# duyhominhnguyen/conan-fgw

Measured on AMD Instinct MI355X. Metric: molecules/s (K=5 conformers), higher is better.
Workload: dtype f32

## Files before the change

### conan-fgw_amd/csrc/fgw_small.hip

```cpp
#include "fgw_common.h"

#ifdef CONAN_FGW_PROFILE
FGW_PROF_ACCESSOR(conan_debug_fgw_prof)
FGW_PROF_TRACE_ACCESSOR(conan_debug_fgw_trace)
#endif

namespace {

constexpr int SK_SCRATCH_DOUBLES = 3 * 256 + 2 * 64;

template <int R, bool KL, bool SECOND = false>
__global__ void __launch_bounds__(FGW_THREADS, (SECOND || R > 9) ? 1 : 3) k_fgw_coupling_small(
    const float *__restrict__ Ys, const float *__restrict__ Cs, const float *__restrict__ ps, const float *__restrict__ pb,
    FgwDims D, conan_fgw_params prm, int outer, int y_zero, const double *__restrict__ Cw, const double *__restrict__ Yw,
    const int *__restrict__ active, float *__restrict__ Tw, int *__restrict__ info, fgw_part_t *__restrict__ Ypart,
    fgw_part_t *__restrict__ Cpart, const double *__restrict__ zvec, const double *__restrict__ yvec, const int *__restrict__ only, FgwAdj adj) {
    extern __shared__ __attribute__((aligned(16))) char smem[];
    auto solve = [&](const int cid) {
    const int b = cid / D.K, s = cid % D.K;
    if (!fgw_active(active, D.B, b, outer)) return;
    const int N = D.N, P = D.P, d = D.d;
    const int NN = N * N, NP = N * P;
    const int tid = threadIdx.x, lane = tid & 63, w = __builtin_amdgcn_readfirstlane(tid >> 6);
    const bool lane_ok = lane < N;
    FGW_PROF_DECL;

    double *Al = reinterpret_cast<double *>(smem);
    double *Gl = Al + NP;
    double *C1l = Gl + NP;
    double *Bl = C1l + NP;
    double *pq = Bl + NP;
    double *red = pq + 128;
    float *t_dummy = reinterpret_cast<float *>(red + 7);
    double *vec4 = red + 8;
    const bool alias = (size_t)NP >= SK_SCRATCH_DOUBLES;
    double *own = vec4 + 256;
    double *bufC = alias ? Al : own;
    double *bufK = bufC + 256;
    double *bufR = bufK + 256;
    double *fcp = bufR + 256;
    double *gcp = fcp + 64;
    float *Tl = reinterpret_cast<float *>(own + (alias ? 0 : SK_SCRATCH_DOUBLES));
    float *C2l = Tl + NP;
    double *Yl = Al;
    float *Zl = reinterpret_cast<float *>(Bl);
    float *Zl2 = reinterpret_cast<float *>(Gl);
    const bool yz_lds = d <= 2 * P;
    const bool z_lds = (size_t)N * d * sizeof(float) <= (size_t)NP * sizeof(double);

    const float *Z = Ys + ((size_t)b * D.K + s) * N * d;
    const float *C2 = adj.rowptr ? adj_dense_slice<FGW_THREADS>(adj, cid, N, tid) : Cs + ((size_t)b * D.K + s) * NN;
    const double *C1 = Cw + (size_t)b * NN;
    const double *Y = Yw + (size_t)b * N * d;
    float *Tg = Tw + ((size_t)b * D.K + s) * NN;
    const double alpha = (double)prm.alpha, inv_eps = 1.0 / (double)prm.epsilon;

    constexpr int EPT = (16 * R * R + FGW_THREADS - 1) / FGW_THREADS;
    double c1v[EPT];
    float c2v[EPT], tv[EPT];
    const bool warm = outer > 0 && prm.warmstart;
#pragma unroll
    for (int u = 0; u < EPT; ++u) {
        const int t = tid + u * FGW_THREADS, tc = t < NN ? t : NN - 1;
        c1v[u] = C1[tc]; c2v[u] = C2[tc]; tv[u] = warm ? Tg[tc] : 0.f;
    }
    const double p_own = tid < N ? (pb ? (double)pb[(size_t)b * N + tid] : 1.0 / (double)N) : 1.0;
    const double q_own = tid < N ? (ps ? (double)ps[((size_t)b * D.K + s) * N + tid] : 1.0 / (double)N) : 1.0;
    double vec_own;
    {
        const int v = tid >> 6, i = tid & 63;
        const double *src = (v == 0 || v == 2) ? yvec + (size_t)b * 2 * N + (v == 0 ? N : 0) : zvec + ((size_t)b * D.K + s) * 2 * N + (v == 1 ? N : 0);
        vec_own = src[i < N ? i : N - 1];
        vec_own = i < N ? vec_own : 0.0;
    }
    const bool stage_yz = yz_lds && !y_zero;
    if (stage_yz) {
        const int Nd = N * d;
        for (int t0 = tid; t0 < Nd; t0 += 4 * FGW_THREADS) {
            double yv[4]; float zv[4];
#pragma unroll
            for (int u = 0; u < 4; ++u) { const int t = t0 + u * FGW_THREADS, tc = t < Nd ? t : Nd - 1; yv[u] = Y[tc]; zv[u] = Z[tc]; }
#pragma unroll
            for (int u = 0; u < 4; ++u) { const int t = t0 + u * FGW_THREADS; if (t < Nd) { Yl[t] = yv[u]; Zl[t] = zv[u]; } }
        }
    }
    if (tid < 64) { pq[tid] = p_own; pq[64 + tid] = q_own; }
    const bool massless = __syncthreads_or(tid < N && (p_own <= 0.0 || q_own <= 0.0)) != 0;
    vec4[tid] = vec_own;
#pragma unroll
    for (int u = 0; u < EPT; ++u) {
        const int t = tid + u * FGW_THREADS;
        if (t < NN) { const int i = t / N, j = t - i * N; C2l[i * P + j] = c2v[u]; if (!stage_yz) C1l[i * P + j] = c1v[u]; }
    }
    __syncthreads();
    FGW_PROF(0);
    const double qj = pq[64 + lane];
    const double pi_l = pq[lane];
#pragma unroll
    for (int u = 0; u < EPT; ++u) {
        const int t = tid + u * FGW_THREADS;
        if (t < NN) { const int i = t / N, j = t - i * N; Tl[i * P + j] = warm ? tv[u] : (float)(pq[i] * pq[64 + j]); }
    }
    const double *r1v = vec4, *r2v = vec4 + 64, *y2v = vec4 + 128, *z2v = vec4 + 192;
    double *Dl = stage_yz ? C1l : Al;
    if (!y_zero) {
        if (stage_yz)
            mm_lds<FGW_WAVES, true>(N, N, d, Yl, d, Zl, d, [&](int i, int j, double v) { Dl[i * P + j] = v; }, border_prepare(N, N));
        else
            mm_f64(N, N, d, [&](int i, int k) { return Y[(size_t)i * d + k]; }, [&](int k, int j) { return (double)Z[(size_t)j * d + k]; },
                   [&](int i, int j, double v) { Dl[i * P + j] = v; });
    }
    __syncthreads();
    FGW_PROF(1);
#pragma unroll
    for (int u = 0; u < EPT; ++u) {
        const int t = tid + u * FGW_THREADS;
        if (t < NN) {
            const int i = t / N, j = t - i * N;
            double m = -2.0 * (y_zero ? 0.0 : Dl[i * P + j]); m += y2v[i]; m += z2v[j];
            m = m > 0.0 ? m : 0.0;
            Bl[i * P + j] = 2.0 * alpha * (r1v[i] + r2v[j]) + (1.0 - alpha) * m;
        }
    }
    __syncthreads();
    if (stage_yz) {
#pragma unroll
        for (int u = 0; u < EPT; ++u) {
            const int t = tid + u * FGW_THREADS;
            if (t < NN) { const int i = t / N, j = t - i * N; C1l[i * P + j] = c1v[u]; }
        }
        __syncthreads();
    }
    FGW_PROF(2);

    const BorderIdx bnn = border_prepare(N, N);
    int cpt = 0, sk_total = 0;
    double err = 1.0;
    while (err > (double)prm.inner_tol && cpt < prm.max_iter) {
        mm_lds<FGW_WAVES, false>(N, N, N, C1l, P, Tl, P, [&](int i, int j, double v) { Al[i * P + j] = v; }, bnn);
        __syncthreads();
        FGW_PROF(3);
        auto product_G = [&]() {
            if constexpr (KL)
                mm_f64(N, N, N, [&](int i, int k) { return Al[i * P + k]; }, [&](int k, int j) { return log((double)C2l[j * P + k] + 1e-15); },
                       [&](int i, int j, double v) { Gl[i * P + j] = v; }, bnn);
            else
                mm_lds<FGW_WAVES, true>(N, N, N, Al, P, C2l, P, [&](int i, int j, double v) { Gl[i * P + j] = 2.0 * v; }, bnn);
        };
        product_G();
        __syncthreads();
        FGW_PROF(4);
        int lq = lane, wq = w;
        asm volatile("" : "+v"(lq), "+v"(wq));
        const int lc = lq < N ? lq : N - 1;
        auto mrA = [&](int r) { const int q = wq + 4 * r, qc = q < N ? q : N - 1; const double m = -(Bl[qc * P + lc] - 2.0 * alpha * Gl[qc * P + lc]) * inv_eps; return (q < N && lane_ok) ? m : -1.0e300; };
        auto mrB = [&](int r) { const int q = wq + 4 * r, qc = q < N ? q : N - 1; const double m = -(Bl[lc * P + qc] - 2.0 * alpha * Gl[lc * P + qc]) * inv_eps; return (q < N && lane_ok) ? m : -1.0e300; };
        double kA[R], kB[R];
        int ii = 0;
        bool exact = massless;
        {
            const double ref_own = -(Bl[lc * P + lc] - 2.0 * alpha * Gl[lc * P + lc]) * inv_eps;
            fcp[lane] = ref_own;
            double cs = 0.0;
#pragma unroll
            for (int r = 0; r < R; ++r) { kA[r] = exp_fast(mrA(r) - ref_own); cs += kA[r]; }
            bufK[w * 64 + lane] = cs;
#pragma unroll
            for (int r = 0; r < R; ++r) { const int q = wq + 4 * r; kB[r] = exp_fast(mrB(r) - fcp[q < N ? q : N - 1]); }
            __syncthreads();
            cs = ((bufK[lane] + bufK[64 + lane]) + bufK[128 + lane]) + bufK[192 + lane];
            if (__any(lane_ok && !(cs > 1e-150 && cs < 1e150))) exact = true;
            const double f = lane_ok ? qj * rcp_pos(cs) : 0.0;
            gcp[lane] = f;
#pragma unroll
            for (int r = 0; r < R; ++r) { kA[r] *= f; kB[r] *= gcp[w + 4 * r]; }
        }
        FGW_PROF(5);
        double colsum = 0.0;
        bool have_colsum = false;
        for (; !exact && ii < prm.num_iter_max; ++ii) {
            if (ii > 0) {
                if (!have_colsum) {
                    double cs = 0.0;
#pragma unroll
                    for (int r = 0; r < R; ++r) cs += kA[r];
                    bufC[w * 64 + lane] = cs;
                    __syncthreads();
                    colsum = ((bufC[lane] + bufC[64 + lane]) + bufC[128 + lane]) + bufC[192 + lane];
                }
                have_colsum = false;
                if (__any(lane_ok && !(colsum > 1e-150 && colsum < 1e150))) { exact = true; break; }
                const double f = lane_ok ? qj * rcp_pos(colsum) : 0.0;
                fcp[lane] = f;
#pragma unroll
                for (int r = 0; r < R; ++r) { kA[r] *= f; kB[r] *= fcp[w + 4 * r]; }
            }
            double rs = 0.0;
#pragma unroll
            for (int r = 0; r < R; ++r) rs += kB[r];
            bufR[w * 64 + lane] = rs;
            __syncthreads();
            rs = ((bufR[lane] + bufR[64 + lane]) + bufR[128 + lane]) + bufR[192 + lane];
            if (__any(lane_ok && !(rs > 1e-150 && rs < 1e150))) { exact = true; break; }
            const double g = lane_ok ? pi_l * rcp_pos(rs) : 0.0;
            gcp[lane] = g;
#pragma unroll
            for (int r = 0; r < R; ++r) { kB[r] *= g; kA[r] *= gcp[w + 4 * r]; }
            if (ii % 10 == 0) {
                double cs = 0.0;
#pragma unroll
                for (int r = 0; r < R; ++r) cs += kA[r];
                bufK[w * 64 + lane] = cs;
                __syncthreads();
                colsum = ((bufK[lane] + bufK[64 + lane]) + bufK[128 + lane]) + bufK[192 + lane];
                have_colsum = true;
                double df = lane_ok ? colsum - qj : 0.0;
                df = wave_sum_d(df * df);
                if (sqrt(df) < (double)prm.stop_thr) { ++ii; break; }
            }
        }
        if (exact) {
            __syncthreads();
            double *xm = bufC, *xs = bufK, *uc = fcp, *vc = gcp;
            const double loga = log(pi_l), logb = log(qj);
            double u_l = 0.0, v_l = 0.0;
            uc[lane] = (lane_ok && !(pi_l > 0.0)) ? loga : 0.0;
            for (ii = 0; ii < prm.num_iter_max; ++ii) {
                double z[R];
                double mx = -1.0e300;
#pragma unroll
                for (int r = 0; r < R; ++r) { z[r] = mrA(r) + uc[w + 4 * r]; mx = fmax(z[r], mx); }
                double sm = 0.0;
#pragma unroll
                for (int r = 0; r < R; ++r) sm += exp_lse(z[r] - mx);
                __syncthreads();
                xm[w * 64 + lane] = mx; xs[w * 64 + lane] = sm;
                __syncthreads();
                {
                    const double m0 = xm[lane], m1 = xm[64 + lane], m2 = xm[128 + lane], m3 = xm[192 + lane];
                    const double M = fmax(fmax(m0, m1), fmax(m2, m3));
                    sm = ((xs[lane] * exp_lse(m0 - M) + xs[64 + lane] * exp_lse(m1 - M)) + xs[128 + lane] * exp_lse(m2 - M)) +
                         xs[192 + lane] * exp_lse(m3 - M);
                    v_l = lane_ok ? logb - (log_acc(sm) + M) : 0.0;
                }
                vc[lane] = v_l;
                mx = -1.0e300;
#pragma unroll
                for (int r = 0; r < R; ++r) { z[r] = mrB(r) + vc[w + 4 * r]; mx = fmax(z[r], mx); }
                sm = 0.0;
#pragma unroll
                for (int r = 0; r < R; ++r) sm += exp_lse(z[r] - mx);
                __syncthreads();
                xm[w * 64 + lane] = mx; xs[w * 64 + lane] = sm;
                __syncthreads();
                {
                    const double m0 = xm[lane], m1 = xm[64 + lane], m2 = xm[128 + lane], m3 = xm[192 + lane];
                    const double M = fmax(fmax(m0, m1), fmax(m2, m3));
                    sm = ((xs[lane] * exp_lse(m0 - M) + xs[64 + lane] * exp_lse(m1 - M)) + xs[128 + lane] * exp_lse(m2 - M)) +
                         xs[192 + lane] * exp_lse(m3 - M);
                    u_l = lane_ok ? loga - (log_acc(sm) + M) : 0.0;
                }
                uc[lane] = u_l;
                if (ii % 10 == 0) {
                    double cs = 0.0;
#pragma unroll
                    for (int r = 0; r < R; ++r) cs += exp_acc(mrA(r) + uc[w + 4 * r] + v_l);
                    __syncthreads();
                    xs[w * 64 + lane] = cs;
                    __syncthreads();
                    cs = ((xs[lane] + xs[64 + lane]) + xs[128 + lane]) + xs[192 + lane];
                    double df = lane_ok ? cs - qj : 0.0;
                    df = wave_sum_d(df * df);
                    if (sqrt(df) < (double)prm.stop_thr) { ++ii; break; }
                }
            }
#pragma unroll
            for (int r = 0; r < R; ++r) kA[r] = exp_acc(mrA(r) + uc[w + 4 * r] + v_l);
        }
        sk_total += ii;
        FGW_PROF(6);
        double e2 = 0.0;
#pragma unroll
        for (int r = 0; r < R; ++r) {
            const int i = wq + 4 * r;
            const bool ok = lane_ok && i < N;
            float *tp = ok ? &Tl[i * P + lq] : t_dummy;
            const float tn = (float)kA[r];
            const double df = ok ? (double)tn - (double)*tp : 0.0;
            e2 += df * df;
            *tp = tn;
        }
        if (cpt % 10 == 0) err = sqrt(block_sum_d(e2, red));
        else __syncthreads();
        ++cpt;
        FGW_PROF(7);
    }
    __syncthreads();
    for (int t = tid; t < NN; t += FGW_THREADS) { const int i = t / N, j = t - i * N; Tg[t] = Tl[i * P + j]; }
    if (tid == 0) { atomicAdd(&info[b * 4 + 1], cpt); atomicAdd(&info[b * 4 + 2], sk_total); }
    FGW_PROF(8);

    if (!prm.fixed_features && Ypart) {
// ... 233 lines not shown
        __syncthreads();
        nb = max(max(ired[0], ired[1]), max(ired[2], ired[3]));
        __syncthreads();
        pad_ok = pad_try && N - nb >= 2 && nb >= 1;
        if (pad_ok) pad_ok = c1_block_ok(nb);
    }
    int m_pad = 0;
    if (pad_try && N - nb >= 2 && nb >= 1) {
        auto nearf = [](double a, double b_) { return fabs(a - b_) <= 1e-9 * (fabs(b_) + 1e-30) || a == b_; };
        bool ok = pad_ok;
        for (int r = nb + 1 + w; r < N; r += FGW_WAVES)
            for (int c = lane; c < d; c += 64) {
                if (stage_yz) {
                    ok = ok && nearf((double)Zl[r * d + c], (double)Zl[nb * d + c]) && nearf(Yl[r * d + c], Yl[nb * d + c]);
                } else {
                    ok = ok && nearf((double)Z[(size_t)r * d + c], (double)Z[(size_t)nb * d + c]);
                    if (!y_zero) ok = ok && nearf(Y[(size_t)r * d + c], Y[(size_t)nb * d + c]);
                }
            }
        if (__syncthreads_and(ok) != 0) m_pad = N - nb;
    }
    const int Nx = m_pad ? nb + 1 : N;
    const double mult = m_pad ? (double)m_pad : 1.0;
    FGW_PROF(0);
    const double qj = pq[64 + lane] * ((m_pad && lane == nb) ? mult : 1.0);
    const double pi_l = pq[lane] * ((m_pad && lane == nb) ? mult : 1.0);
    const double *r1v = vec4, *r2v = vec4 + 64, *y2v = vec4 + 128, *z2v = vec4 + 192;
    auto base_of = [&](int i, int j, double dot) {
        double m = -2.0 * dot; m += y2v[i]; m += z2v[j];
        m = m > 0.0 ? m : 0.0;
        return fc.two_alpha * (r1v[i] + r2v[j]) + fc.one_m_alpha * m;
    };
    if (y_zero) {
        int i = e_i0, j = e_j0;
#pragma unroll
        for (int u = 0; u < EPT; ++u) {
            if (tid + u * FGW_THREADS < NN) Bl[i * P + j] = base_of(i, j, 0.0);
            j += e_dr; i += e_dq;
            if (j >= N) { j -= N; ++i; }
        }
    } else if (stage_yz) {
        mm_lds2<FGW_WAVES, MAXT, 0, true, true>(Nx, Nx, d, Yl, d, Zl, d, [&]() { load_c1_t(); __syncthreads(); },
                                                [&](int i, int j, double v) { Bl[i * P + j] = base_of(i, j, v); });
        for_entries([&](int u, int o) { C1l[o] = c1v[u]; });
    } else {
        mm_f64(Nx, Nx, d, [&](int i, int k) { return Y[(size_t)i * d + k]; }, [&](int k, int j) { return (double)Z[(size_t)j * d + k]; },
               [&](int i, int j, double v) { Bl[i * P + j] = base_of(i, j, v); });
    }
    __syncthreads();
    FGW_PROF(1);
    if (warm) {
        if (m_pad) {
            int i = e_i0, j = e_j0;
#pragma unroll
            for (int u = 0; u < EPT; ++u) {
                if (tid + u * FGW_THREADS < NN) Tl[i * P + j] = (float)((double)tv[u] * ((i == nb ? mult : 1.0) * (j == nb ? mult : 1.0)));
                j += e_dr; i += e_dq;
                if (j >= N) { j -= N; ++i; }
            }
        } else {
            for_entries([&](int u, int o) { Tl[o] = tv[u]; });
        }
    } else {
#pragma unroll
        for (int r = 0; r < R; ++r) {
            const int i = w + 4 * r;
            const double pi_r = (pb ? (double)pb[(size_t)b * N + (i < N ? i : N - 1)] : fc.inv_n) * ((m_pad && i == nb) ? mult : 1.0);
            if (i < Nx && lane < Nx) Tl[i * P + lane] = (float)(pi_r * qj);
        }
    }
    __syncthreads();
    FGW_PROF(2);

    int cpt = 0, sk_total = 0;
    double err = 1.0;
    bool bail = __syncthreads_or(tid < N && (p_own <= 0.0 || q_own <= 0.0)) != 0;
    while (!bail && err > fc.inner_tol && cpt < prm.max_iter) {
        int tq = tid, N = Nx, P = D.P;
        asm volatile("" : "+v"(tq), "+s"(N), "+s"(P));
        int nbq = m_pad ? nb : -1;
        asm volatile("" : "+s"(nbq));
        const int lq = tq & 63, wq = tq >> 6;
        const bool lq_ok = lq < N;
        mm_lds2<FGW_WAVES, 1, 0, false, false>(N, N, N, C1l, P, Tl, P, [] {}, [&](int i, int j, double v) { AKl[i * P + j] = v; }, tq);
        __syncthreads();
        FGW_PROF(3);
        int nr = n_real;
        asm volatile("" : "+s"(nr));
        if (complete) {
            {
                const int lc = lq_ok ? lq : N - 1;
                const double *ar = AKl + lc * P + wq;
                double p0 = 0.0, p1 = 0.0;
#pragma unroll
                for (int r = 0; r < R; ++r) {
                    const int q = wq + 4 * r;
                    if (q < nr) { if (r & 1) p1 += ar[4 * r]; else p0 += ar[4 * r]; }
                }
                if (lq_ok) rsum[wq * N + lq] = p0 + p1;
            }
            __syncthreads();
            {
                int i = tq / N, j = tq - i * N;
                const int dq = FGW_THREADS / N, dr = FGW_THREADS - dq * N;
                for (int t = tq; t < N * N; t += FGW_THREADS) {
                    const int o = i * P + j;
                    const double ai = ((rsum[i] + rsum[N + i]) + rsum[2 * N + i]) + rsum[3 * N + i];
                    const double v = j < nr ? ai - AKl[o] : 0.0;
                    const double x = fma(v, fc.four_alpha_inv_eps, (Bl[j * P + j] - Bl[o]) * fc.inv_eps);
                    AKl[o] = exp_fast(x);
                    j += dr; i += dq;
                    if (j >= N) { j -= N; ++i; }
                }
            }
        } else {
            mm_lds2<FGW_WAVES, MAXT, 0, true, true>(N, N, N, AKl, P, C2l, P, [&]() { __syncthreads(); }, [&](int i, int j, double v) {
                const double x = fma(v, fc.four_alpha_inv_eps, (Bl[j * P + j] - Bl[i * P + j]) * fc.inv_eps);
                AKl[i * P + j] = exp_fast(x);
            }, tq);
        }
        __syncthreads();
        FGW_PROF(4);
        double kA[R], kB[R];
        {
            const int lc = lq_ok ? lq : N - 1;
#pragma unroll
            for (int r = 0; r < R; ++r) {
                const int q = wq + 4 * r, qc = q < N ? q : N - 1;
                const double a = AKl[qc * P + lc], bb = AKl[lc * P + qc];
                const bool ok = q < N && lq_ok;
                kA[r] = ok ? a : 0.0; kB[r] = ok ? bb : 0.0;
            }
        }
        __syncthreads();
        FGW_PROF(5);
        const int permL = (lq & 3) * 16 + (lq >> 2);
        double *bufCw = bufC + wq * 64 + lq, *bufRw = bufR + wq * 64 + lq;
        const double *fw = fvP + wq * 16, *gw = gvP + wq * 16;
        auto dotR = [&](const double (&k)[R], const double *v) {
            double p0 = 0.0, p1 = 0.0, p2 = 0.0;
#pragma unroll
            for (int r = 0; r < R; ++r) {
                if (r % 3 == 0) p0 = fma(k[r], v[r], p0);
                else if (r % 3 == 1) p1 = fma(k[r], v[r], p1);
                else p2 = fma(k[r], v[r], p2);
            }
            return (p0 + p1) + p2;
        };
        int ii = 0;
        double f = 0.0, g = 0.0, colp = 0.0;
        bool have_colp = false;
        for (; ii < prm.num_iter_max; ++ii) {
            if (!have_colp) {
                double pc = 0.0;
                if (ii == 0) {
                    gvP[permL] = lq_ok ? (lq == nbq ? (double)m_pad : 1.0) : 0.0;
                }
                pc = dotR(kA, gw);
                *bufCw = pc;
                __syncthreads();
                colp = ((bufC[lq] + bufC[64 + lq]) + bufC[128 + lq]) + bufC[192 + lq];
            }
            have_colp = false;
            if (__any(lq_ok && !(colp > 1e-150 && colp < 1e150))) { bail = true; break; }
            f = lq_ok ? qj * rcp_pos(colp) : 0.0;
            fvP[permL] = f;
            *bufRw = dotR(kB, fw);
            __syncthreads();
            const double rs = ((bufR[lq] + bufR[64 + lq]) + bufR[128 + lq]) + bufR[192 + lq];
            if (__any(lq_ok && !(rs > 1e-150 && rs < 1e150))) { bail = true; break; }
            g = lq_ok ? pi_l * rcp_pos(rs) : 0.0;
            gvP[permL] = g;
            if (ii % 10 == 0) {
                *bufCw = dotR(kA, gw);
                __syncthreads();
                colp = ((bufC[lq] + bufC[64 + lq]) + bufC[128 + lq]) + bufC[192 + lq];
                have_colp = true;
                double df = lq_ok ? f * colp - qj : 0.0;
                df = df * df;
                if (lq == nbq) df /= (double)m_pad;
                df = wave_sum_d(df);
                if (sqrt(df) < fc.stop_thr) { ++ii; break; }
            }
        }
        if (bail) break;
        sk_total += ii;
        FGW_PROF(6);
        double e2 = 0.0;
        {
            float *trow = Tl + wq * P + lq;
#pragma unroll
            for (int r = 0; r < R; ++r) {
                const bool ok = lq_ok && wq + 4 * r < N;
                float *tp = ok ? trow + 4 * r * P : t_dummy;
                const float tn = (float)((gw[r] * kA[r]) * f);
                double df = ok ? (double)tn - (double)*tp : 0.0;
                df *= df;
                if (nbq >= 0) {
                    const double im = 1.0 / (double)m_pad;
                    df *= (lq == nbq ? im : 1.0) * (wq + 4 * r == nbq ? im : 1.0);
                }
                e2 += df;
                *tp = tn;
            }
        }
        if (cpt % 10 == 0) err = sqrt(block_sum_d(e2, red));
        else __syncthreads();
        ++cpt;
        FGW_PROF(7);
    }
    if (bail) {
        if (tid == 0) { redo[cid] = 1; atomicOr(&info[b * 4 + 3], 1); }
        return;
    }
    __syncthreads();
    {
        int te = tid;
        asm volatile("" : "+v"(te));
        int i = te / N, j = te - i * N;
        const int dq = FGW_THREADS / N, dr = FGW_THREADS - dq * N;
        if (m_pad) {
            const float im = (float)(1.0 / mult);
            for (int t = te; t < NN; t += FGW_THREADS) {
                Tg[t] = Tl[min(i, nb) * P + min(j, nb)] * ((i >= nb ? im : 1.0f) * (j >= nb ? im : 1.0f));
                j += dr; i += dq;
                if (j >= N) { j -= N; ++i; }
            }
        } else {
            for (int t = te; t < NN; t += FGW_THREADS) {
                Tg[t] = Tl[i * P + j];
                j += dr; i += dq;
                if (j >= N) { j -= N; ++i; }
            }
        }
    }
    if (tid == 0) { atomicAdd(&info[b * 4 + 1], cpt); atomicAdd(&info[b * 4 + 2], sk_total); redo[cid] = 0; if (m_pad) atomicOr(&info[b * 4 + 3], 2); }
    FGW_PROF(8);

    if (!prm.fixed_features && Ypart) {
        fgw_part_t *Yp = Ypart + ((size_t)b * D.K + s) * N * d;
        if (yz_lds) {
            const int Nd = N * d;
            for (int t0 = tid; t0 < Nd; t0 += 4 * FGW_THREADS) {
                float zv[4];
#pragma unroll
                for (int u = 0; u < 4; ++u) { const int t = t0 + u * FGW_THREADS; zv[u] = Z[t < Nd ? t : Nd - 1]; }
#pragma unroll
                for (int u = 0; u < 4; ++u) { const int t = t0 + u * FGW_THREADS; if (t < Nd) Zl[t] = zv[u]; }
            }
            __syncthreads();
            mm_lds2<FGW_WAVES, 1, 0, false, false>(N, d, N, Tl, P, Zl, d, [] {}, [&](int i, int c, double v) { Yp[(size_t)i * d + c] = (fgw_part_t)v; });
        } else {
            mm_f64(N, d, N, [&](int i, int k) { return (double)Tl[i * P + k]; }, [&](int k, int c) { return (double)Z[(size_t)k * d + c]; },
                   [&](int i, int c, double v) { Yp[(size_t)i * d + c] = (fgw_part_t)v; });
        }
    }
    FGW_PROF(9);
    if (!prm.fixed_structure) {
        fgw_part_t *Cp = Cpart + ((size_t)b * D.K + s) * NN;
        if (complete) {
            {
                const int lc = lane < Nx ? lane : Nx - 1;
                const float *tr = Tl + lc * P + w;
                double p0 = 0.0, p1 = 0.0;
#pragma unroll
                for (int r = 0; r < R; ++r) {
                    const int q = w + 4 * r;
                    if (q < n_real) { if (r & 1) p1 += (double)tr[4 * r]; else p0 += (double)tr[4 * r]; }
                }
                if (lane < Nx) rsum[w * N + lane] = p0 + p1;
            }
            __syncthreads();
            mm_lds2<FGW_WAVES, 1, 0, true, false>(Nx, Nx, n_real, Tl, P, Tl, P, [] {}, [&](int i, int j, double v) {
                const double ti = ((rsum[i] + rsum[N + i]) + rsum[2 * N + i]) + rsum[3 * N + i];
                const double tj = ((rsum[j] + rsum[N + j]) + rsum[2 * N + j]) + rsum[3 * N + j];
                if (m_pad) Bl[i * P + j] = ti * tj - v;
                else Cp[i * N + j] = (fgw_part_t)(ti * tj - v);
            });
        } else {
            mm_lds2<FGW_WAVES, 1, 0, false, false>(Nx, Nx, Nx, Tl, P, C2l, P, [] {}, [&](int i, int j, double v) { AKl[i * P + j] = v; });
            __syncthreads();
            mm_lds2<FGW_WAVES, 1, 0, true, false>(Nx, Nx, Nx, AKl, P, Tl, P, [] {}, [&](int i, int j, double v) {
                if (m_pad) Bl[i * P + j] = v;
                else Cp[i * N + j] = (fgw_part_t)v;
            });
        }
        if (m_pad) {
            __syncthreads();
            const double im = 1.0 / mult;
            int i = tid / N, j = tid - i * N;
            const int dq = FGW_THREADS / N, dr = FGW_THREADS - dq * N;
            for (int t = tid; t < NN; t += FGW_THREADS) {
                Cp[t] = (fgw_part_t)(Bl[min(i, nb) * P + min(j, nb)] * ((i >= nb ? im : 1.0) * (j >= nb ? im : 1.0)));
                j += dr; i += dq;
                if (j >= N) { j -= N; ++i; }
            }
        }
    }
    FGW_PROF(10);
    FGW_PROF_FLUSH;
    FGW_PROF_TRACE(Nx | (cpt << 8) | (sk_total << 20));
}

template <int NT>
__device__ __forceinline__ void molecule_vectors(const double *__restrict__ Y, const double *__restrict__ C, const float *__restrict__ p, int N,
                                                 int d, bool kl, double *__restrict__ out, int which = 2) {
    constexpr int LPI = NT / 64;
    const int i = (int)threadIdx.x / LPI, sub = (int)threadIdx.x % LPI;
    double y2 = 0.0, r1 = 0.0;
    if (i < N) {
        if (which != 1)
            for (int c = sub; c < d; c += LPI) { const double v = Y[(size_t)i * d + c]; y2 += v * v; }
        if (which != 0)
            for (int k = sub; k < N; k += LPI) {
                const double c1 = C[i * N + k], pk = p ? (double)p[k] : 1.0 / (double)N;
                r1 += (kl ? c1 * log(c1 + 1e-15) - c1 : c1 * c1) * pk;
            }
    }
#pragma unroll
    for (int o = 1; o < LPI; o <<= 1) { y2 += __shfl_xor(y2, o, 64); r1 += __shfl_xor(r1, o, 64); }
    if (i < N && sub == 0) { if (which != 1) out[i] = y2; if (which != 0) out[N + i] = r1; }
}

__global__ void __launch_bounds__(256) k_fgw_small_vectors(const float *__restrict__ Ys, const float *__restrict__ Cs, const float *__restrict__ ps,
                                                           const float *__restrict__ pb, FgwDims D, int kl, double *__restrict__ Cw,
                                                           double *__restrict__ Yw, double *__restrict__ zvec, double *__restrict__ yvec,
                                                           const float *__restrict__ init_C, const float *__restrict__ init_Y, int max_iter,
                                                           int *__restrict__ active, int *__restrict__ info, float *__restrict__ errs,
                                                           float *__restrict__ Yout, float *__restrict__ Cout, FgwAdj adj) {
    const int b = blockIdx.x / D.K, s = blockIdx.x % D.K;
    const int N = D.N, d = D.d;
    __shared__ __attribute__((aligned(16))) unsigned char cm[64 * 65 + 16];
    const int Pm = D.P;
    if (adj.rowptr) {
        for (int t = threadIdx.x; t < (64 * 65 + 16) / 4; t += 256) reinterpret_cast<unsigned *>(cm)[t] = 0u;
        __syncthreads();
        adj_scatter_lds_bytes<256>(adj, (int)blockIdx.x, N, Pm, cm, (int)threadIdx.x);
        __syncthreads();
    }
    if (s == 0) {
        const int NN = N * N, Nd = N * d;
        const float *c0 = init_C ? init_C + (size_t)b * NN : Cs + (size_t)b * D.K * NN;
        for (int t = threadIdx.x; t < NN; t += 256) {
            const float cv = (!init_C && adj.rowptr) ? (float)cm[(t / N) * Pm + (t % N)] : c0[t];
            Cw[(size_t)b * NN + t] = (double)cv; Cout[(size_t)b * NN + t] = cv;
        }
        for (int t = threadIdx.x; t < Nd; t += 256) {
            const float y = init_Y ? init_Y[(size_t)b * Nd + t] : 0.f;
            Yw[(size_t)b * Nd + t] = (double)y; Yout[(size_t)b * Nd + t] = y;
        }
        if (threadIdx.x == 0) { fgw_active_init(active, D.B, b); info[b * 4 + 0] = 0; info[b * 4 + 1] = 0; info[b * 4 + 2] = 0; info[b * 4 + 3] = 0; }
        for (int t = threadIdx.x; t < 2 * max_iter; t += 256) errs[(size_t)b * 2 * max_iter + t] = __builtin_nanf("");
        __syncthreads();
    }
    const float *Z = Ys + ((size_t)b * D.K + s) * N * d;
    const float *C2 = Cs + ((size_t)b * D.K + s) * N * N;
    const float *q = ps ? ps + ((size_t)b * D.K + s) * N : nullptr;
    const int j = (int)threadIdx.x >> 2, sub = (int)threadIdx.x & 3;
    double z2 = 0.0, r2 = 0.0;
    if (j < N) {
        for (int c = sub; c < d; c += 4) { const double v = (double)Z[(size_t)j * d + c]; z2 += v * v; }
        for (int k = sub; k < N; k += 4) {
            const double c2 = adj.rowptr ? (double)cm[j * Pm + k] : (double)C2[j * N + k], qk = q ? (double)q[k] : 1.0 / (double)N;
            r2 += qk * (kl ? c2 : c2 * c2);
        }
    }
    z2 += __shfl_xor(z2, 1, 64); z2 += __shfl_xor(z2, 2, 64);
    r2 += __shfl_xor(r2, 1, 64); r2 += __shfl_xor(r2, 2, 64);
    double *zo = zvec + ((size_t)b * D.K + s) * 2 * N;
    if (j < N && sub == 0) { zo[j] = z2; zo[N + j] = r2; }
    if (s == 0)
        molecule_vectors<256>(Yw + (size_t)b * N * d, Cw + (size_t)b * N * N, pb ? pb + (size_t)b * N : nullptr, N, d, kl != 0, yvec + (size_t)b * 2 * N);
    if (adj.order && blockIdx.x == gridDim.x - 1) fgw_order_by_size<256>(adj, D.B, D.K, (int)threadIdx.x);
}

constexpr int UPD_THREADS = 512;
template <bool Y_FROM_T>
__global__ void __launch_bounds__(UPD_THREADS) k_fgw_update_parts(
    const float *__restrict__ pb, const float *__restrict__ lambdas, FgwDims D, conan_fgw_params prm, int outer,
    const fgw_part_t *__restrict__ Ypart, const fgw_part_t *__restrict__ Cpart, double *__restrict__ Cw, double *__restrict__ Yw,
    int *__restrict__ active, int *__restrict__ info, float *__restrict__ errs, float *__restrict__ Yout, float *__restrict__ Cout,
    double *__restrict__ yvec, const float *__restrict__ Tw, const float *__restrict__ Ys, int chunk) {
    __shared__ double red[UPD_THREADS / 64 + 1];
    extern __shared__ __attribute__((aligned(16))) char usmem[];
    const int part = (int)blockIdx.x >= D.B ? 1 : 0;
    const int b = (int)blockIdx.x - part * D.B;
    const int N = D.N, d = D.d, K = D.K, NN = N * N, Nd = N * d;
    const int tid = threadIdx.x;
    int *flag_out = active + (outer & 1) * 2 * D.B + part * D.B + b;
    if (!fgw_active(active, D.B, b, outer)) {
        if (tid == 0) *flag_out = 0;
        return;
    }
    constexpr int U = 4;
    double e2 = 0.0;
    if (part == 0) {
        if (!prm.fixed_features) {
            double *Yb = Yw + (size_t)b * Nd;
            if constexpr (Y_FROM_T) {
                float *Tl = reinterpret_cast<float *>(usmem), *Zl = Tl + (size_t)chunk * NN;
                const int lane = tid & 63, wave = __builtin_amdgcn_readfirstlane(tid >> 6), li = lane & 15, lk = lane >> 4;
                const int Mq = (N + 15) >> 4, Nq = (d + 15) >> 4;
                constexpr int NWU = UPD_THREADS / 64, TW = 2;
                for (int t0 = 0; t0 < Mq * Nq; t0 += NWU * TW) {
                    int ti0[TW], tj0[TW], tic[TW], tjc[TW];
                    bool mine[TW];
                    f64x4 sum[TW];
#pragma unroll
                    for (int w = 0; w < TW; ++w) {
                        const int t = t0 + wave + w * NWU;
                        mine[w] = t < Mq * Nq;
                        ti0[w] = mine[w] ? (t / Nq) << 4 : 0; tj0[w] = mine[w] ? (t % Nq) << 4 : 0;
                        tic[w] = min(ti0[w] + li, N - 1); tjc[w] = min(tj0[w] + li, d - 1);
                        sum[w] = f64x4{0.0, 0.0, 0.0, 0.0};
                    }
                    for (int s0 = 0; s0 < K; s0 += chunk) {
                        const int cs = min(chunk, K - s0);
                        __syncthreads();
                        const float *tg = Tw + ((size_t)b * K + s0) * NN, *zg = Ys + ((size_t)b * K + s0) * Nd;
                        auto stage = [&](const float *__restrict__ src, float *dst, int n) {
                            constexpr int SB = 12;
                            for (int base = 0; base < n; base += SB * UPD_THREADS) {
                                float v[SB];
#pragma unroll
                                for (int u = 0; u < SB; ++u) { const int q = base + u * UPD_THREADS + tid; v[u] = src[q < n ? q : n - 1]; }
#pragma unroll
                                for (int u = 0; u < SB; ++u) { const int q = base + u * UPD_THREADS + tid; if (q < n) dst[q] = v[u]; }
                            }
                        };
                        stage(tg, Tl, cs * NN);
                        stage(zg, Zl, cs * Nd);
                        __syncthreads();
#pragma unroll
                        for (int w = 0; w < TW; ++w)
                            if (mine[w])
                                for (int q = 0; q < cs; ++q) {
                                    const double lam = lambdas ? (double)lambdas[s0 + q] : 1.0 / (double)K;
                                    const f64x4 r = mm2_tile<0, false>(Tl + (size_t)q * NN + tic[w] * N + lk, Zl + (size_t)q * Nd + lk * d + tjc[w], d, N, lk);
                                    sum[w] = sum[w] + lam * r;
                                }
                    }
#pragma unroll
                    for (int w = 0; w < TW; ++w) {
                        const int jb = tj0[w] + li;
                        if (mine[w] && jb < d) {
#pragma unroll
                            for (int qq = 0; qq < 4; ++qq) {
                                const int i = ti0[w] + lk + 4 * qq;
                                if (i < N) {
                                    const double pw = pb ? (double)pb[(size_t)b * N + i] : 1.0 / (double)N;
                                    const double yn = sum[w][qq] * (pw > 0.0 ? 1.0 / pw : 0.0);
                                    const double df = yn - Yb[i * d + jb];
                                    e2 += df * df;
                                    Yb[i * d + jb] = yn;
                                    Yout[(size_t)b * Nd + i * d + jb] = (float)yn;
                                }
                            }
                        }
                    }
                }
            } else {
                for (int t0 = tid; t0 < Nd; t0 += U * UPD_THREADS) {
                    double acc[U], old[U];
#pragma unroll
                    for (int u = 0; u < U; ++u) {
                        const int t = t0 + u * UPD_THREADS;
                        acc[u] = 0.0; old[u] = 0.0;
                        if (t < Nd) {
                            old[u] = Yb[t];
                            for (int s = 0; s < K; ++s) {
                                const double lam = lambdas ? (double)lambdas[s] : 1.0 / (double)K;
                                const int i = t / d;
                                const double pw = pb ? (double)pb[(size_t)b * N + i] : 1.0 / (double)N;
                                const double pinv = pw > 0.0 ? 1.0 / pw : 0.0;
                                acc[u] += lam * Ypart[((size_t)b * K + s) * Nd + t] * pinv;
                            }
                        }
                    }
#pragma unroll
                    for (int u = 0; u < U; ++u) {
                        const int t = t0 + u * UPD_THREADS;
                        if (t < Nd) {
                            const double df = acc[u] - old[u];
                            e2 += df * df;
                            Yb[t] = acc[u];
                            Yout[(size_t)b * Nd + t] = (float)acc[u];
                        }
                    }
                }
            }
        }
    } else if (!prm.fixed_structure) {
        double *Cb = Cw + (size_t)b * NN;
        for (int t0 = tid; t0 < NN; t0 += U * UPD_THREADS) {
            double acc[U], old[U];
#pragma unroll
            for (int u = 0; u < U; ++u) {
                const int t = t0 + u * UPD_THREADS;
                acc[u] = 0.0; old[u] = 0.0;
                if (t < NN) {
                    old[u] = Cb[t];
                    for (int s = 0; s < K; ++s) {
                        const double lam = lambdas ? (double)lambdas[s] : 1.0 / (double)K;
                        acc[u] += lam * Cpart[((size_t)b * K + s) * NN + t];
                    }
                }
            }
#pragma unroll
            for (int u = 0; u < U; ++u) {
                const int t = t0 + u * UPD_THREADS;
                if (t < NN) {
                    const int i = t / N, j = t - i * N;
                    const double pi = pb ? (double)pb[(size_t)b * N + i] : 1.0 / (double)N;
                    const double pj = pb ? (double)pb[(size_t)b * N + j] : 1.0 / (double)N;
                    const double cn = pi * pj > 0.0 ? (prm.loss_fun ? exp(acc[u] / (pi * pj)) : acc[u] / (pi * pj)) : 0.0;
                    const double df = cn - old[u];
                    e2 += df * df;
                    Cb[t] = cn;
                    Cout[(size_t)b * NN + t] = (float)cn;
                }
            }
        }
    }
    const double err = sqrt(block_sum_d<UPD_THREADS / 64>(e2, red));
    if (yvec) molecule_vectors<UPD_THREADS>(Yw + (size_t)b * Nd, Cw + (size_t)b * NN, pb ? pb + (size_t)b * N : nullptr, N, d, prm.loss_fun != 0,
                                            yvec + (size_t)b * 2 * N, part);
    if (tid == 0) {
        errs[((size_t)b * 2 + part) * prm.max_iter + outer] = (float)err;
        info[b * 4 + 0] = outer + 1;
        *flag_out = err > (double)prm.tol ? 1 : 0;
    }
}

inline size_t small_lds(int N, int d) {
    const size_t NP = (size_t)N * fgw_pitch(N);
    (void)d; return NP * 8 * 4 + (256 + 128 + 8 + (NP >= (size_t)SK_SCRATCH_DOUBLES ? 0 : SK_SCRATCH_DOUBLES)) * 8 + NP * 4 * 2;
}

}

bool conan_fgw_small_supported(int N, int d) { return N <= 64 && small_lds(N, d) <= 160 * 1024; }

void conan_fgw_small_prepare(const FgwCall &c) {
    k_fgw_small_vectors<<<c.D.B * c.D.K, 256, 0, c.s>>>(c.Ys, c.Cs, c.ps, c.p, c.D, c.prm.loss_fun, c.Cw, c.Yw, c.zvec, c.yvec, c.init_C, c.init_Y,
                                                       c.prm.max_iter, c.active, c.info, c.errs, c.Y, c.C, c.adj);
}

template <class F>
static void with_rows(int R, F &&f) {
    if (R <= 6) f(std::integral_constant<int, 6>{});
    else if (R <= 9) f(std::integral_constant<int, 9>{});
    else if (R <= 12) f(std::integral_constant<int, 12>{});
    else f(std::integral_constant<int, 16>{});
}

template <int R, typename C2T>
static void launch_fast(const FgwCall &c, int outer, int y_zero, fgw_part_t *Ypart) {
    const FgwDims &D = c.D;
    const int tpw = fast_tiles_per_wave(D.N);
    auto go = [&](auto kernel) {
        launch_lds(kernel, D.B * D.K, FGW_THREADS, fast_lds<C2T>(D.N).bytes, c.s, c.Ys, c.Cs, c.ps, c.p, D, c.prm, fast_const(c.prm, D.N), outer,
                   y_zero, c.Cw, c.Yw, c.active, c.T, c.info, Ypart, c.Cpart, c.zvec, c.yvec, c.redo, c.adj);
    };
    if constexpr (R <= 6) go(k_fgw_coupling_fast<R, 1, C2T>);
    else if constexpr (R <= 12) { if (tpw <= 1) go(k_fgw_coupling_fast<R, 1, C2T>); else go(k_fgw_coupling_fast<R, 3, C2T>); }
    else { if (tpw <= 1) go(k_fgw_coupling_fast<R, 1, C2T>); else if (tpw <= 3) go(k_fgw_coupling_fast<R, 3, C2T>); else go(k_fgw_coupling_fast<R, 4, C2T>); }
}

bool conan_fgw_fast_supported(int N, int d, int small_int) {
    if (N > 64 || N < 4) return false;
    const size_t lds = small_int ? fast_lds<unsigned char>(N).bytes : fast_lds<float>(N).bytes;
    return lds <= 160 * 1024 && d >= 1;
}

void conan_fgw_small_coupling(const FgwCall &c, int outer, int y_zero, fgw_part_t *Ypart) {
    const FgwDims &D = c.D;
    const size_t lds = small_lds(D.N, D.d);
    const int grid = D.B * D.K;
    const bool kl = c.prm.loss_fun != 0;
    with_rows((D.N + 3) / 4, [&](auto R) {
        const int *only = nullptr;
        if (!kl && conan_fgw_fast_supported(D.N, D.d, c.prm.cs_small_int)) {
            if (c.prm.cs_small_int) launch_fast<R.value, unsigned char>(c, outer, y_zero, Ypart);
            else launch_fast<R.value, float>(c, outer, y_zero, Ypart);
            only = c.redo;
        }
        auto exact = [&](auto kernel, int blocks) {
            launch_lds(kernel, blocks, FGW_THREADS, lds, c.s, c.Ys, c.Cs, c.ps, c.p, D, c.prm, outer, y_zero, c.Cw, c.Yw, c.active, c.T, c.info, Ypart,
                       c.Cpart, c.zvec, c.yvec, only, c.adj);
        };
        if (kl) exact(k_fgw_coupling_small<R.value, true, false>, grid);
        else if (only) exact(k_fgw_coupling_small<R.value, false, true>, (grid + 63) / 64);
        else exact(k_fgw_coupling_small<R.value, false, false>, grid);
    });
}

void conan_fgw_small_update(const FgwCall &c, int outer, bool y_from_t) {
    const FgwDims &D = c.D;
    const int chunk = y_from_t ? conan_fgw_update_chunk(D.K, D.N, D.d, D.B) : 0;
    if (chunk > 0)
        launch_lds(k_fgw_update_parts<true>, 2 * D.B, UPD_THREADS, (size_t)chunk * ((size_t)D.N * D.N + (size_t)D.N * D.d) * 4, c.s, c.p, c.lambdas, D,
                   c.prm, outer, nullptr, c.Cpart, c.Cw, c.Yw, c.active, c.info, c.errs, c.Y, c.C, c.yvec, c.T, c.Ys, chunk);
    else
        k_fgw_update_parts<false><<<2 * D.B, UPD_THREADS, 0, c.s>>>(c.p, c.lambdas, D, c.prm, outer, c.Ypart, c.Cpart, c.Cw, c.Yw, c.active, c.info, c.errs,
                                                                     c.Y, c.C, c.yvec, nullptr, nullptr, 0);
}

int conan_fgw_update_chunk(int K, int N, int d, int B) {
    if (N > 64) return 0;
    const size_t per = ((size_t)N * N + (size_t)N * d) * 4, budget = (2 * B <= 256 ? 144 : 72) * 1024;
    if (per > budget) return 0;
    const int c = (int)(budget / per);
    return c < K ? c : K;
}
```

Before: 116,800.

## Async LDS staging in update kernel, LDS-sourced molecule vectors, prefetch before active check

The update kernel now stages T and Z chunks into LDS with global_load_lds async copies, and issues the first chunk before the active check so the load overlaps the early work. Updated Y and C values are also written to LDS so molecule_vectors reads them from LDS rather than re-reading global doubles. The C-part reduction batches Cpart loads across conformers. The prepare kernel moves the order-by-size work to a dedicated extra block, computes molecule vectors straight from the inputs and drops a barrier. Together these add LDS footprint and complexity in exchange for less serialized global traffic and shorter critical paths.

```diff
diff --git a/conan-fgw_amd/csrc/fgw_small.hip b/conan-fgw_amd/csrc/fgw_small.hip
--- a/conan-fgw_amd/csrc/fgw_small.hip
+++ b/conan-fgw_amd/csrc/fgw_small.hip
@@ -1,3 +1,4 @@
+#include <algorithm>
 #include "fgw_common.h"
 
 #ifdef CONAN_FGW_PROFILE
@@ -837,24 +838,29 @@
     FGW_PROF_TRACE(Nx | (cpt << 8) | (sk_total << 20));
 }
 
-template <int NT>
-__device__ __forceinline__ void molecule_vectors(const double *__restrict__ Y, const double *__restrict__ C, const float *__restrict__ p, int N,
-                                                 int d, bool kl, double *__restrict__ out, int which = 2) {
+template <int NT, class FY, class FC>
+__device__ __forceinline__ void molecule_vectors_of(FY Y, FC C, const float *__restrict__ p, int N, int d, bool kl, double *__restrict__ out,
+                                                 int which = 2) {
     constexpr int LPI = NT / 64;
     const int i = (int)threadIdx.x / LPI, sub = (int)threadIdx.x % LPI;
     double y2 = 0.0, r1 = 0.0;
     if (i < N) {
         if (which != 1)
-            for (int c = sub; c < d; c += LPI) { const double v = Y[(size_t)i * d + c]; y2 += v * v; }
+            for (int c = sub; c < d; c += LPI) { const double v = Y(i, c); y2 += v * v; }
         if (which != 0)
             for (int k = sub; k < N; k += LPI) {
-                const double c1 = C[i * N + k], pk = p ? (double)p[k] : 1.0 / (double)N;
+                const double c1 = C(i, k), pk = p ? (double)p[k] : 1.0 / (double)N;
                 r1 += (kl ? c1 * log(c1 + 1e-15) - c1 : c1 * c1) * pk;
             }
     }
 #pragma unroll
     for (int o = 1; o < LPI; o <<= 1) { y2 += __shfl_xor(y2, o, 64); r1 += __shfl_xor(r1, o, 64); }
     if (i < N && sub == 0) { if (which != 1) out[i] = y2; if (which != 0) out[N + i] = r1; }
+}
+template <int NT>
+__device__ __forceinline__ void molecule_vectors(const double *__restrict__ Y, const double *__restrict__ C, const float *__restrict__ p, int N,
+                                                 int d, bool kl, double *__restrict__ out, int which = 2) {
+    molecule_vectors_of<NT>([&](int i, int c) { return Y[(size_t)i * d + c]; }, [&](int i, int k) { return C[i * N + k]; }, p, N, d, kl, out, which);
 }
 
 __global__ void __launch_bounds__(256) k_fgw_small_vectors(const float *__restrict__ Ys, const float *__restrict__ Cs, const float *__restrict__ ps,
@@ -863,21 +869,24 @@
                                                            const float *__restrict__ init_C, const float *__restrict__ init_Y, int max_iter,
                                                            int *__restrict__ active, int *__restrict__ info, float *__restrict__ errs,
                                                            float *__restrict__ Yout, float *__restrict__ Cout, FgwAdj adj) {
-    const int b = blockIdx.x / D.K, s = blockIdx.x % D.K;
+    if (adj.order && blockIdx.x == 0) { fgw_order_by_size<256>(adj, D.B, D.K, (int)threadIdx.x); return; }
+    const int g = (int)blockIdx.x - (adj.order ? 1 : 0);
+    const int b = g / D.K, s = g % D.K;
     const int N = D.N, d = D.d;
     __shared__ __attribute__((aligned(16))) unsigned char cm[64 * 65 + 16];
     const int Pm = D.P;
     if (adj.rowptr) {
         for (int t = threadIdx.x; t < (64 * 65 + 16) / 4; t += 256) reinterpret_cast<unsigned *>(cm)[t] = 0u;
         __syncthreads();
-        adj_scatter_lds_bytes<256>(adj, (int)blockIdx.x, N, Pm, cm, (int)threadIdx.x);
+        adj_scatter_lds_bytes<256>(adj, g, N, Pm, cm, (int)threadIdx.x);
         __syncthreads();
     }
+    const int NN = N * N, Nd = N * d;
+    const float *c0 = init_C ? init_C + (size_t)b * NN : Cs + (size_t)b * D.K * NN;
+    const bool c_lds = !init_C && adj.rowptr;
     if (s == 0) {
-        const int NN = N * N, Nd = N * d;
-        const float *c0 = init_C ? init_C + (size_t)b * NN : Cs + (size_t)b * D.K * NN;
         for (int t = threadIdx.x; t < NN; t += 256) {
-            const float cv = (!init_C && adj.rowptr) ? (float)cm[(t / N) * Pm + (t % N)] : c0[t];
+            const float cv = c_lds ? (float)cm[(t / N) * Pm + (t % N)] : c0[t];
             Cw[(size_t)b * NN + t] = (double)cv; Cout[(size_t)b * NN + t] = cv;
         }
         for (int t = threadIdx.x; t < Nd; t += 256) {
@@ -886,7 +895,6 @@
         }
         if (threadIdx.x == 0) { fgw_active_init(active, D.B, b); info[b * 4 + 0] = 0; info[b * 4 + 1] = 0; info[b * 4 + 2] = 0; info[b * 4 + 3] = 0; }
         for (int t = threadIdx.x; t < 2 * max_iter; t += 256) errs[(size_t)b * 2 * max_iter + t] = __builtin_nanf("");
-        __syncthreads();
     }
     const float *Z = Ys + ((size_t)b * D.K + s) * N * d;
     const float *C2 = Cs + ((size_t)b * D.K + s) * N * N;
@@ -905,17 +913,44 @@
     double *zo = zvec + ((size_t)b * D.K + s) * 2 * N;
     if (j < N && sub == 0) { zo[j] = z2; zo[N + j] = r2; }
     if (s == 0)
-        molecule_vectors<256>(Yw + (size_t)b * N * d, Cw + (size_t)b * N * N, pb ? pb + (size_t)b * N : nullptr, N, d, kl != 0, yvec + (size_t)b * 2 * N);
-    if (adj.order && blockIdx.x == gridDim.x - 1) fgw_order_by_size<256>(adj, D.B, D.K, (int)threadIdx.x);
+        molecule_vectors_of<256>([&](int i, int c) { return (double)(init_Y ? init_Y[(size_t)b * Nd + (size_t)i * d + c] : 0.f); },
+                                 [&](int i, int k) { return (double)(c_lds ? (float)cm[i * Pm + k] : c0[i * N + k]); },
+                                 pb ? pb + (size_t)b * N : nullptr, N, d, kl != 0, yvec + (size_t)b * 2 * N);
 }
 
 constexpr int UPD_THREADS = 512;
+__host__ __device__ inline int upd_pad64(int n) { return (n + 63) & ~63; }
+constexpr int UPD_KB = 5;
+#ifdef CONAN_FGW_PROFILE
+#define UPD_PROF_DECL long long uprof_t = wall_clock64(); long long uprof_acc[5] = {0, 0, 0, 0, 0}
+#define UPD_PROF(k) do { const long long t_ = wall_clock64(); uprof_acc[k] += t_ - uprof_t; uprof_t = t_; } while (0)
+#define UPD_PROF_FLUSH(base)                                                                                                                         \
+    do {                                                                                                                                             \
+        if (threadIdx.x == 0) {                                                                                                                      \
+            for (int k_ = 0; k_ < 5; ++k_) atomicAdd(reinterpret_cast<unsigned long long *>(&g_fgw_prof[(base) + k_]), (unsigned long long)uprof_acc[k_]); \
+            atomicAdd(reinterpret_cast<unsigned long long *>(&g_fgw_prof[(base) + 5]), 1ull);                                                        \
+        }                                                                                                                                            \
+    } while (0)
+#else
+#define UPD_PROF_DECL
+#define UPD_PROF(k)
+#define UPD_PROF_FLUSH(base)
+#endif
+__device__ __forceinline__ void upd_stage(const float *__restrict__ tg, int nt, const float *__restrict__ zg, int nz, float *Tl, float *Zl, int tid) {
+    const int lane = tid & 63, wave = __builtin_amdgcn_readfirstlane(tid >> 6);
+    for (int q0 = wave * 64; q0 < nt; q0 += UPD_THREADS)
+        __builtin_amdgcn_global_load_lds((const __attribute__((address_space(1))) void *)(tg + min(q0 + lane, nt - 1)),
+                                         (__attribute__((address_space(3))) void *)(Tl + q0), 4, 0, 0);
+    for (int q0 = wave * 64; q0 < nz; q0 += UPD_THREADS)
+        __builtin_amdgcn_global_load_lds((const __attribute__((address_space(1))) void *)(zg + min(q0 + lane, nz - 1)),
+                                         (__attribute__((address_space(3))) void *)(Zl + q0), 4, 0, 0);
+}
 template <bool Y_FROM_T>
-__global__ void __launch_bounds__(UPD_THREADS) k_fgw_update_parts(
+__global__ void __launch_bounds__(UPD_THREADS, 4) k_fgw_update_parts(
     const float *__restrict__ pb, const float *__restrict__ lambdas, FgwDims D, conan_fgw_params prm, int outer,
     const fgw_part_t *__restrict__ Ypart, const fgw_part_t *__restrict__ Cpart, double *__restrict__ Cw, double *__restrict__ Yw,
     int *__restrict__ active, int *__restrict__ info, float *__restrict__ errs, float *__restrict__ Yout, float *__restrict__ Cout,
-    double *__restrict__ yvec, const float *__restrict__ Tw, const float *__restrict__ Ys, int chunk) {
+    double *__restrict__ yvec, const float *__restrict__ Tw, const float *__restrict__ Ys, int chunk, int y_off) {
     __shared__ double red[UPD_THREADS / 64 + 1];
     extern __shared__ __attribute__((aligned(16))) char usmem[];
     const int part = (int)blockIdx.x >= D.B ? 1 : 0;
@@ -923,17 +958,28 @@
     const int N = D.N, d = D.d, K = D.K, NN = N * N, Nd = N * d;
     const int tid = threadIdx.x;
     int *flag_out = active + (outer & 1) * 2 * D.B + part * D.B + b;
+    UPD_PROF_DECL;
+    const bool y_here = Y_FROM_T && part == 0 && !prm.fixed_features;
+    auto stage = [&](int s0, int cs) {
+        float *Tl = reinterpret_cast<float *>(usmem), *Zl = Tl + upd_pad64(chunk * NN);
+        upd_stage(Tw + ((size_t)b * K + s0) * NN, cs * NN, Ys + ((size_t)b * K + s0) * Nd, cs * Nd, Tl, Zl, tid);
+    };
+    if constexpr (Y_FROM_T) { if (y_here) stage(0, min(chunk, K)); }
     if (!fgw_active(active, D.B, b, outer)) {
+        if constexpr (Y_FROM_T) { if (y_here) asm volatile("s_waitcnt vmcnt(0)" ::: "memory"); }
         if (tid == 0) *flag_out = 0;
         return;
     }
+    UPD_PROF(0);
     constexpr int U = 4;
     double e2 = 0.0;
+    double *Yl = nullptr, *Cl = nullptr;
     if (part == 0) {
         if (!prm.fixed_features) {
             double *Yb = Yw + (size_t)b * Nd;
             if constexpr (Y_FROM_T) {
-                float *Tl = reinterpret_cast<float *>(usmem), *Zl = Tl + (size_t)chunk * NN;
+                float *Tl = reinterpret_cast<float *>(usmem), *Zl = Tl + upd_pad64(chunk * NN);
+                if (y_off >= 0) Yl = reinterpret_cast<double *>(usmem + y_off);
                 const int lane = tid & 63, wave = __builtin_amdgcn_readfirstlane(tid >> 6), li = lane & 15, lk = lane >> 4;
                 const int Mq = (N + 15) >> 4, Nq = (d + 15) >> 4;
                 constexpr int NWU = UPD_THREADS / 64, TW = 2;
@@ -951,21 +997,13 @@
                     }
                     for (int s0 = 0; s0 < K; s0 += chunk) {
                         const int cs = min(chunk, K - s0);
+                        if (!y_here || t0 > 0 || s0 > 0) {
+                            __syncthreads();
+                            stage(s0, cs);
+                        }
+                        asm volatile("s_waitcnt vmcnt(0)" ::: "memory");
                         __syncthreads();
-                        const float *tg = Tw + ((size_t)b * K + s0) * NN, *zg = Ys + ((size_t)b * K + s0) * Nd;
-                        auto stage = [&](const float *__restrict__ src, float *dst, int n) {
-                            constexpr int SB = 12;
-                            for (int base = 0; base < n; base += SB * UPD_THREADS) {
-                                float v[SB];
-#pragma unroll
-                                for (int u = 0; u < SB; ++u) { const int q = base + u * UPD_THREADS + tid; v[u] = src[q < n ? q : n - 1]; }
-#pragma unroll
-                                for (int u = 0; u < SB; ++u) { const int q = base + u * UPD_THREADS + tid; if (q < n) dst[q] = v[u]; }
-                            }
-                        };
-                        stage(tg, Tl, cs * NN);
-                        stage(zg, Zl, cs * Nd);
-                        __syncthreads();
+                        UPD_PROF(1);
 #pragma unroll
                         for (int w = 0; w < TW; ++w)
                             if (mine[w])
@@ -975,6 +1013,8 @@
                                     sum[w] = sum[w] + lam * r;
                                 }
                     }
+                    __syncthreads();
+                    UPD_PROF(2);
 #pragma unroll
                     for (int w = 0; w < TW; ++w) {
                         const int jb = tj0[w] + li;
@@ -989,6 +1029,7 @@
                                     e2 += df * df;
                                     Yb[i * d + jb] = yn;
                                     Yout[(size_t)b * Nd + i * d + jb] = (float)yn;
+                                    if (Yl) Yl[i * d + jb] = yn;
                                 }
                             }
                         }
@@ -1027,17 +1068,46 @@
         }
     } else if (!prm.fixed_structure) {
         double *Cb = Cw + (size_t)b * NN;
+        if constexpr (Y_FROM_T) Cl = reinterpret_cast<double *>(usmem);
         for (int t0 = tid; t0 < NN; t0 += U * UPD_THREADS) {
             double acc[U], old[U];
-#pragma unroll
-            for (int u = 0; u < U; ++u) {
-                const int t = t0 + u * UPD_THREADS;
-                acc[u] = 0.0; old[u] = 0.0;
-                if (t < NN) {
-                    old[u] = Cb[t];
-                    for (int s = 0; s < K; ++s) {
-                        const double lam = lambdas ? (double)lambdas[s] : 1.0 / (double)K;
-                        acc[u] += lam * Cpart[((size_t)b * K + s) * NN + t];
+            [[maybe_unused]] float pif[U], pjf[U];
+            if constexpr (Y_FROM_T) {
+                int tc[U];
+#pragma unroll
+                for (int u = 0; u < U; ++u) {
+                    tc[u] = min(t0 + u * UPD_THREADS, NN - 1);
+                    const int i = tc[u] / N, j = tc[u] - i * N;
+                    acc[u] = 0.0;
+                    old[u] = Cb[tc[u]];
+                    pif[u] = pb ? pb[(size_t)b * N + i] : 0.f;
+                    pjf[u] = pb ? pb[(size_t)b * N + j] : 0.f;
+                }
+                for (int s0 = 0; s0 < K; s0 += UPD_KB) {
+                    double cv[UPD_KB][U];
+#pragma unroll
+                    for (int q = 0; q < UPD_KB; ++q)
+#pragma unroll
+                        for (int u = 0; u < U; ++u) cv[q][u] = Cpart[((size_t)b * K + min(s0 + q, K - 1)) * NN + tc[u]];
+#pragma unroll
+                    for (int q = 0; q < UPD_KB; ++q)
+                        if (s0 + q < K) {
+                            const double lam = lambdas ? (double)lambdas[s0 + q] : 1.0 / (double)K;
+#pragma unroll
+                            for (int u = 0; u < U; ++u) acc[u] += lam * cv[q][u];
+                        }
+                }
+            } else {
+#pragma unroll
+                for (int u = 0; u < U; ++u) {
+                    const int t = t0 + u * UPD_THREADS;
+                    acc[u] = 0.0; old[u] = 0.0;
+                    if (t < NN) {
+                        old[u] = Cb[t];
+                        for (int s = 0; s < K; ++s) {
+                            const double lam = lambdas ? (double)lambdas[s] : 1.0 / (double)K;
+                            acc[u] += lam * Cpart[((size_t)b * K + s) * NN + t];
+                        }
                     }
                 }
             }
@@ -1045,26 +1115,39 @@
             for (int u = 0; u < U; ++u) {
                 const int t = t0 + u * UPD_THREADS;
                 if (t < NN) {
-                    const int i = t / N, j = t - i * N;
-                    const double pi = pb ? (double)pb[(size_t)b * N + i] : 1.0 / (double)N;
-                    const double pj = pb ? (double)pb[(size_t)b * N + j] : 1.0 / (double)N;
+                    double pi, pj;
+                    if constexpr (Y_FROM_T) {
+                        pi = pb ? (double)pif[u] : 1.0 / (double)N;
+                        pj = pb ? (double)pjf[u] : 1.0 / (double)N;
+                    } else {
+                        const int i = t / N, j = t - i * N;
+                        pi = pb ? (double)pb[(size_t)b * N + i] : 1.0 / (double)N;
+                        pj = pb ? (double)pb[(size_t)b * N + j] : 1.0 / (double)N;
+                    }
                     const double cn = pi * pj > 0.0 ? (prm.loss_fun ? exp(acc[u] / (pi * pj)) : acc[u] / (pi * pj)) : 0.0;
                     const double df = cn - old[u];
                     e2 += df * df;
                     Cb[t] = cn;
                     Cout[(size_t)b * NN + t] = (float)cn;
-                }
-            }
-        }
-    }
+                    if constexpr (Y_FROM_T) Cl[t] = cn;
+                }
+            }
+        }
+    }
+    UPD_PROF(3);
     const double err = sqrt(block_sum_d<UPD_THREADS / 64>(e2, red));
-    if (yvec) molecule_vectors<UPD_THREADS>(Yw + (size_t)b * Nd, Cw + (size_t)b * NN, pb ? pb + (size_t)b * N : nullptr, N, d, prm.loss_fun != 0,
-                                            yvec + (size_t)b * 2 * N, part);
+    if (yvec) {
+        const float *pm = pb ? pb + (size_t)b * N : nullptr;
+        if (Yl || Cl) molecule_vectors<UPD_THREADS>(Yl, Cl, pm, N, d, prm.loss_fun != 0, yvec + (size_t)b * 2 * N, part);
+        else molecule_vectors<UPD_THREADS>(Yw + (size_t)b * Nd, Cw + (size_t)b * NN, pm, N, d, prm.loss_fun != 0, yvec + (size_t)b * 2 * N, part);
+    }
     if (tid == 0) {
         errs[((size_t)b * 2 + part) * prm.max_iter + outer] = (float)err;
         info[b * 4 + 0] = outer + 1;
         *flag_out = err > (double)prm.tol ? 1 : 0;
     }
+    UPD_PROF(4);
+    UPD_PROF_FLUSH(part ? 22 : 11);
 }
 
 inline size_t small_lds(int N, int d) {
@@ -1077,7 +1160,7 @@
 bool conan_fgw_small_supported(int N, int d) { return N <= 64 && small_lds(N, d) <= 160 * 1024; }
 
 void conan_fgw_small_prepare(const FgwCall &c) {
-    k_fgw_small_vectors<<<c.D.B * c.D.K, 256, 0, c.s>>>(c.Ys, c.Cs, c.ps, c.p, c.D, c.prm.loss_fun, c.Cw, c.Yw, c.zvec, c.yvec, c.init_C, c.init_Y,
+    k_fgw_small_vectors<<<c.D.B * c.D.K + (c.adj.order ? 1 : 0), 256, 0, c.s>>>(c.Ys, c.Cs, c.ps, c.p, c.D, c.prm.loss_fun, c.Cw, c.Yw, c.zvec, c.yvec, c.init_C, c.init_Y,
                                                        c.prm.max_iter, c.active, c.info, c.errs, c.Y, c.C, c.adj);
 }
 
@@ -1133,12 +1216,18 @@
 void conan_fgw_small_update(const FgwCall &c, int outer, bool y_from_t) {
     const FgwDims &D = c.D;
     const int chunk = y_from_t ? conan_fgw_update_chunk(D.K, D.N, D.d, D.B) : 0;
-    if (chunk > 0)
-        launch_lds(k_fgw_update_parts<true>, 2 * D.B, UPD_THREADS, (size_t)chunk * ((size_t)D.N * D.N + (size_t)D.N * D.d) * 4, c.s, c.p, c.lambdas, D,
-                   c.prm, outer, nullptr, c.Cpart, c.Cw, c.Yw, c.active, c.info, c.errs, c.Y, c.C, c.yvec, c.T, c.Ys, chunk);
+    if (chunk > 0) {
+        const size_t stage = ((size_t)upd_pad64(chunk * D.N * D.N) + (size_t)upd_pad64(chunk * D.N * D.d)) * 4, ybytes = (size_t)D.N * D.d * 8, cbytes = (size_t)D.N * D.N * 8;
+        const bool one_round = ((D.N + 15) / 16) * ((D.d + 15) / 16) <= 2 * (UPD_THREADS / 64);
+        const size_t with_y = one_round ? std::max(stage, ybytes) : (stage + 15) / 16 * 16 + ybytes;
+        const bool y_lds = with_y <= (2 * D.B <= 256 ? 156 : 78) * (size_t)1024;
+        const int y_off = y_lds ? (one_round ? 0 : (int)((stage + 15) / 16 * 16)) : -1;
+        launch_lds(k_fgw_update_parts<true>, 2 * D.B, UPD_THREADS, std::max(y_lds ? with_y : stage, cbytes), c.s, c.p, c.lambdas, D,
+                   c.prm, outer, nullptr, c.Cpart, c.Cw, c.Yw, c.active, c.info, c.errs, c.Y, c.C, c.yvec, c.T, c.Ys, chunk, y_off);
+    }
     else
         k_fgw_update_parts<false><<<2 * D.B, UPD_THREADS, 0, c.s>>>(c.p, c.lambdas, D, c.prm, outer, c.Ypart, c.Cpart, c.Cw, c.Yw, c.active, c.info, c.errs,
-                                                                     c.Y, c.C, c.yvec, nullptr, nullptr, 0);
+                                                                     c.Y, c.C, c.yvec, nullptr, nullptr, 0, -1);
 }
 
 int conan_fgw_update_chunk(int K, int N, int d, int B) {
```

Result: no change. 117,900 (median of 6 runs) (+1.0%).
